# cggos/ptam_cg

Measured on AMD Instinct MI355X. Metric: BA LM iterations/s (50 KF x 5k pts) [+ tracked frames/s @640x480 in 'tracking'], higher is better.
Workload: dtype f64; 1 GPU; bundle_50kf_x_5000pts_dense; keyframes=50, points_total=5000, measurements_total=250000, measurements_rank0=250000, estimator=Tukey, parallelism=1 GPU, halfsample=R

## Files before the change

### ptam_cg_amd/csrc/ba_schur.inc

```
__device__ __forceinline__ void vinv_body(const BaDev& d, double lambda, int bx) {
    const int p = bx * 256 + threadIdx.x;
    if (p >= d.P) return;
    double v[6];
    const int r0 = d.rowptr[p], r1 = d.rowptr[p + 1];
    const int c0 = r0 >> 6, c1 = (r1 - 1) >> 6;
    if (d.cut != nullptr && r1 > r0 && c0 != c1) {
        const double* q = d.cut + (size_t)(2 * c0 + 1) * 9;
        double e[3] = {q[6], q[7], q[8]};
#pragma unroll
        for (int i = 0; i < 6; i++) v[i] = q[i];
        for (int c = c0 + 1; c <= c1; c++) {
            q = d.cut + (size_t)(2 * c) * 9;
#pragma unroll
            for (int i = 0; i < 6; i++) v[i] += q[i];
#pragma unroll
            for (int i = 0; i < 3; i++) e[i] += q[6 + i];
        }
#pragma unroll
        for (int i = 0; i < 3; i++) d.epsB[(size_t)p * 3 + i] = e[i];
    } else {
#pragma unroll
        for (int i = 0; i < 6; i++) v[i] = d.V[(size_t)p * 6 + i];
    }
    double A[9] = {v[0], v[1], v[3], v[1], v[2], v[4], v[3], v[4], v[5]};
    double* out = d.Vinv + (size_t)p * 9;
    if (A[0] * A[4] * A[8] == 0) {
#pragma unroll
        for (int i = 0; i < 9; i++) out[i] = 0;
        return;
    }
    A[0] *= (1.0 + lambda);
    A[4] *= (1.0 + lambda);
    A[8] *= (1.0 + lambda);
    for (int col = 0; col < 3; col++) {
        double inv_diag = 1;
        for (int row = col; row < 3; row++) {
            double val = A[row * 3 + col];
            for (int c2 = 0; c2 < col; c2++) val -= A[c2 * 3 + col] * A[row * 3 + c2];
            if (row == col) {
                A[row * 3 + col] = val;
                inv_diag = 1 / val;
            } else {
                A[col * 3 + row] = val;
                A[row * 3 + col] = val * inv_diag;
            }
        }
    }
    for (int c = 0; c < 3; c++) {
        double y[3], x[3];
        for (int i = 0; i < 3; i++) {
            double val = (i == c) ? 1.0 : 0.0;
            for (int j = 0; j < i; j++) val -= A[i * 3 + j] * y[j];
            y[i] = val;
        }
        for (int i = 0; i < 3; i++) y[i] /= A[i * 3 + i];
        for (int i = 2; i >= 0; i--) {
            double val = y[i];
            for (int j = i + 1; j < 3; j++) val -= A[j * 3 + i] * x[j];
            x[i] = val;
        }
        for (int r = 0; r < 3; r++) out[r * 3 + c] = x[r];
    }
}

__global__ void __launch_bounds__(256) vinv_kernel(BaDev d, double lambda) {
    TL_MARK(d, 6)
    if (ba_guard_blocks(d)) return;
    vinv_body(d, lambda, blockIdx.x);
}
__global__ void __launch_bounds__(256) reduce_vinv_kernel(BaDev d, int grid_acc, int nx, double lambda, double lambda_stay) {
    TL_MARK(d, 5)
    const int4 gf = ba_guard_load(d);
    if (ba_guard_blocks(d, gf)) return;
    if (ba_guard_stay(d, gf)) lambda = lambda_stay;
    const int b = blockIdx.x, nr = nx * RSPLIT;
    if (b < nr)
        reduce_partials_body(d, grid_acc, b % nx, b / nx);
    else
        vinv_body(d, lambda, b - nr);
}

#define SCHUR_TILE_ELEMS (SCHUR_TC * SCHUR_TC * 36 + SCHUR_TC * 6)
#ifndef SCHUR_RING
#define SCHUR_RING 2
#endif
#ifndef SCHUR_NW
#define SCHUR_NW 4
#endif
#define SCHUR_WG_PER_CU (8 / SCHUR_NW)
#define SCHUR_RED_BYTES ((SCHUR_NW / 2) * 40 * 64 * 8)
#define SCHUR_N_VARIANTS 6
#define SCHUR_MAP_WPT 8

struct SchurGrp {
    double wa[3][3];
    double wb[3][3];
    double vi[9];
    double eb[3];
    unsigned pm;
};
typedef double v4f64 __attribute__((ext_vector_type(4)));
typedef double schur_d2 __attribute__((ext_vector_type(2), aligned(8)));

template <int MODE>
__host__ __device__ __forceinline__ int schur_row(int t, int rid) {
    if (MODE == 1) return rid;
    if (t < 2) return 6 * (rid / 3) + 2 * (rid % 3) + t;
    const int q = 16 + (rid >> 1);
    return 6 * (q / 3) + 2 * (q % 3) + (rid & 1);
}
struct SchurLane {
    int hi4, sh4, hi2, sh2;
    unsigned o4, o2;
};
template <int MODE>
__device__ __forceinline__ SchurLane schur_lane(int l15) {
    SchurLane L;
    const int r0 = schur_row<MODE>(0, l15), r2 = MODE == 3 ? schur_row<3>(2, l15) : 0;
    const int s0 = r0 / 6, s2 = r2 / 6;
    L.hi4 = s0 >> 2, L.sh4 = 8 * (s0 & 3), L.o4 = 8u * (unsigned)(r0 - 6 * s0);
    L.hi2 = s2 >> 2, L.sh2 = 8 * (s2 & 3), L.o2 = 8u * (unsigned)(r2 - 6 * s2);
    return L;
}

__device__ __forceinline__ unsigned schur_slot_off(unsigned o0, unsigned o1, int first, int hi, int sh, int M, bool& present) {
    const unsigned o = ((hi ? o1 : o0) >> sh) & 0xffu;
    present = o != 0xffu;
    return (present ? (unsigned)first + o : (unsigned)M) * 48u;
}

template <int MODE>
__device__ __forceinline__ void schur_fetch_role(const char* __restrict__ W0, const char* __restrict__ W1, const char* __restrict__ W2,
// ... 494 lines not shown
```

### ptam_cg_amd/csrc/ba_update.inc

```
__global__ void __launch_bounds__(64) pose_update_kernel(BaDev d, int cur) {
    const int c = blockIdx.x * 64 + threadIdx.x;
    if (c < d.C) {
        const double* T = d.pose[cur] + 12 * c;
        double* Tn = d.pose[cur ^ 1] + 12 * c;
        const int f = d.cam_free[c];
        if (f < 0) {
#pragma unroll
            for (int i = 0; i < 12; i++) Tn[i] = T[i];
        } else {
            double mu[6], Tl[12], o[12];
#pragma unroll
            for (int i = 0; i < 6; i++) mu[i] = d.da[6 * f + i];
#pragma unroll
            for (int i = 0; i < 12; i++) Tl[i] = T[i];
            se3_exp_mul(mu, Tl, o);
#pragma unroll
            for (int i = 0; i < 12; i++) Tn[i] = o[i];
        }
    }
    if (blockIdx.x == 0) {
        double s = 0;
        for (int i = threadIdx.x; i < d.n; i += 64) s += d.da[i] * d.da[i];
        s = wave_sum_f64(s);
        if (threadIdx.x == 0) d.sumsq2[0] = s, d.sumsq2[1] = 0.0;
// ... 34 lines not shown
                t2 += w[(2 * h) * 3 + 2] * a0 + w[(2 * h + 1) * 3 + 2] * a1;
            }
        }
    }
    Ts[tid][0] = t0, Ts[tid][1] = t1, Ts[tid][2] = t2;
    __syncthreads();
    if (tid < 64) {
        double s0 = 0, s1 = 0, s2 = 0;
        for (int q = tid; q < BA_CHUNK; q += 64) s0 += Ts[q][0], s1 += Ts[q][1], s2 += Ts[q][2];
        s0 = wave_sum_f64(s0), s1 = wave_sum_f64(s1), s2 = wave_sum_f64(s2);
        if (tid == 0) {
            const double* eb = d.epsB + (size_t)pp * 3;
            const double* vi = d.Vinv + (size_t)pp * 9;
            const double* X = d.pt[cur] + (size_t)pp * 3;
            const double v0 = eb[0] - s0, v1 = eb[1] - s1, v2 = eb[2] - s2;
            const double d0 = vi[0] * v0 + vi[1] * v1 + vi[2] * v2, d1 = vi[3] * v0 + vi[4] * v1 + vi[5] * v2, d2 = vi[6] * v0 + vi[7] * v1 + vi[8] * v2;
            double* Xn = d.pt[cur ^ 1] + (size_t)pp * 3;
            Xn[0] = X[0] + d0, Xn[1] = X[1] + d1, Xn[2] = X[2] + d2;
            wred[0][0] = Xn[0], wred[0][1] = Xn[1], wred[1][0] = Xn[2], wred[1][1] = d0 * d0 + d1 * d1 + d2 * d2;
        }
    }
    __syncthreads();
    const double Xn[3] = {wred[0][0], wred[0][1], wred[1][0]};
    const double sq = wred[1][1];
    const double s2 = sig2;
    double err = 0;
    for (int m = ch.m_begin + tid; m < ch.m_end; m += BA_CHUNK) {
        if (d.m_state[m] == MS_DEAD) continue;
        BaProj pr;
        if (!ba_project(cam, d.pose[cur ^ 1] + 12 * d.m_cam[m], Xn, pr)) {
            err += 1.0;
            d.m_zbad_t[m] = 1;
        } else {
            const double2 fo = d.m_found[m];
            const double sn = d.m_s[m];
            const double ex = sn * (fo.x - pr.u), ey = sn * (fo.y - pr.v), e2n = ex * ex + ey * ey;
            err += ba_objective(est, e2n, s2, 1.0 / s2);
            d.m_e2t[m] = e2n;
            d.m_zbad_t[m] = 0;
        }
    }
    __syncthreads();
    err = wave_sum_f64(err);
    if ((tid & 63) == 0) wred[tid >> 6][0] = err;
    __syncthreads();
    if (tid == 0) {
        double e = 0;
        for (int i = 0; i < BA_CHUNK / 64; i++) e += wred[i][0];
        d.err_part[2 * blockIdx.x] = e;
        d.err_part[2 * blockIdx.x + 1] = sq;
    }
}

template <bool LOADW>
__global__ void __launch_bounds__(BA_CHUNK) point_update_kernel(DevCam cam, BaDev d, int cur, int est) {
    TL_MARK(d, 11)
    __shared__ double Ts[BA_CHUNK][3];
    __shared__ double Np[BA_CHUNK][3];
    __shared__ double wred[BA_CHUNK / 64][2];
    const int tid = threadIdx.x;
    const BaChunk ch = d.chunks[blockIdx.x];
    if (ch.m_end - ch.m_begin > BA_CHUNK) {
        point_update_long<LOADW>(cam, d, cur, est, ch, Ts, wred);
        return;
    }
    const int m = ch.m_begin + tid;
    const bool active = m < ch.m_end;
    const int mc = min(m, d.M - 1);
    const int st = active ? (int)d.m_state[mc] : (int)MS_DEAD;
    const int c = d.m_cam[mc], p = d.m_pt[mc];
    const int f = d.m_fidx[mc];
    const double s2 = d.sc->sigma_sq;
    const double2 fo = d.m_found[mc];
    const double sn = d.m_s[mc];
    const int npts = ch.pt_end - ch.pt_begin;
    const int pi0 = tid >> 3, sub = tid & 7;
    const bool on0 = pi0 < npts;
    const int pp0 = ch.pt_begin + (on0 ? pi0 : 0);
    const int rq0 = d.rowptr[pp0], rq1 = d.rowptr[pp0 + 1];
    double vi[9], x[3], eb[3];
    {
        const double* Vi = d.Vinv + (size_t)pp0 * 9;
        const double* X = d.pt[cur] + (size_t)pp0 * 3;
        const double* E = d.epsB + (size_t)pp0 * 3;
#pragma unroll
        for (int i = 0; i < 9; i++) vi[i] = Vi[i];
#pragma unroll
        for (int i = 0; i < 3; i++) x[i] = X[i], eb[i] = E[i];
    }
    double w[18];
    if (LOADW) {
        const size_t wp = w_plane(d);
#pragma unroll
        for (int c3 = 0; c3 < 3; c3++)
#pragma unroll
            for (int h = 0; h < 3; h++) {
                const double2 t = *(const double2*)(d.W + c3 * wp + (size_t)mc * 6 + 2 * h);
                w[(2 * h) * 3 + c3] = t.x;
                w[(2 * h + 1) * 3 + c3] = t.y;
            }
    }
    double da[6], T[12], Tc[12], xm[3];
    {
        const double2* dq = (const double2*)(d.da + 6 * (size_t)max(f, 0));
        const double2* Tq = (const double2*)(d.pose[cur ^ 1] + 12 * (size_t)c);
        if (!LOADW) {
            const double2* Cq = (const double2*)(d.pose[cur] + 12 * (size_t)c);
            const double* Xm = d.pt[cur] + (size_t)p * 3;
#pragma unroll
            for (int i = 0; i < 6; i++) {
                const double2 t = Cq[i];
                Tc[2 * i] = t.x, Tc[2 * i + 1] = t.y;
            }
#pragma unroll
            for (int i = 0; i < 3; i++) xm[i] = Xm[i];
        }
#pragma unroll
        for (int i = 0; i < 3; i++) {
            const double2 t = dq[i];
            da[2 * i] = t.x, da[2 * i + 1] = t.y;
        }
        if (LOADW) {
#pragma unroll
            for (int i = 0; i < 6; i++) {
                const double2 t = Tq[i];
                T[2 * i] = t.x, T[2 * i + 1] = t.y;
            }
        }
    }
    double t0 = 0, t1 = 0, t2 = 0;
    if (st == MS_ALIVE && f >= 0) {
        if (!LOADW) ba_rebuild_w(cam, est, Tc, xm, fo, sn, s2, w);
#pragma unroll
        for (int r = 0; r < 6; r++) {
            const double a = da[r];
            t0 += w[r * 3] * a;
            t1 += w[r * 3 + 1] * a;
            t2 += w[r * 3 + 2] * a;
        }
    }
    if (!LOADW) {
        const double2* Tq = (const double2*)(d.pose[cur ^ 1] + 12 * (size_t)c);
#pragma unroll
        for (int i = 0; i < 6; i++) {
            const double2 t = Tq[i];
            T[2 * i] = t.x, T[2 * i + 1] = t.y;
        }
    }
    Ts[tid][0] = t0;
    Ts[tid][1] = t1;
    Ts[tid][2] = t2;
    __syncthreads();
    double sq = 0;
    for (int base = 0; base < npts; base += BA_CHUNK / 8) {
        const int pi = base + pi0;
        const bool on = pi < npts;
        const int pp = ch.pt_begin + (on ? pi : 0);
        int r0 = rq0 - ch.m_begin, r1 = on0 ? rq1 - ch.m_begin : r0;
        if (base != 0) {
            r0 = d.rowptr[pp] - ch.m_begin, r1 = on ? d.rowptr[pp + 1] - ch.m_begin : r0;
            const double* Vi = d.Vinv + (size_t)pp * 9;
            const double* X = d.pt[cur] + (size_t)pp * 3;
            const double* E = d.epsB + (size_t)pp * 3;
#pragma unroll
            for (int i = 0; i < 9; i++) vi[i] = Vi[i];
#pragma unroll
            for (int i = 0; i < 3; i++) x[i] = X[i], eb[i] = E[i];
        }
        const double e0 = eb[0], e1 = eb[1], e2 = eb[2];
        double s0 = 0, s1 = 0, s2 = 0;
        for (int rr = r0 + sub; rr < r1; rr += 8) {
            s0 += Ts[rr][0];
            s1 += Ts[rr][1];
            s2 += Ts[rr][2];
        }
        s0 += dpp_row_shr_f64<1>(s0), s1 += dpp_row_shr_f64<1>(s1), s2 += dpp_row_shr_f64<1>(s2);
        s0 += dpp_row_shr_f64<2>(s0), s1 += dpp_row_shr_f64<2>(s1), s2 += dpp_row_shr_f64<2>(s2);
        s0 += dpp_row_shr_f64<4>(s0), s1 += dpp_row_shr_f64<4>(s1), s2 += dpp_row_shr_f64<4>(s2);
        if (on && sub == 7) {
            const double v0 = e0 - s0, v1 = e1 - s1, v2 = e2 - s2;
            const double d0 = vi[0] * v0 + vi[1] * v1 + vi[2] * v2;
            const double d1 = vi[3] * v0 + vi[4] * v1 + vi[5] * v2;
            const double d2 = vi[6] * v0 + vi[7] * v1 + vi[8] * v2;
            sq += d0 * d0 + d1 * d1 + d2 * d2;
            const double n0 = x[0] + d0, n1 = x[1] + d1, n2 = x[2] + d2;
            double* Xn = d.pt[cur ^ 1] + (size_t)pp * 3;
            Xn[0] = n0;
            Xn[1] = n1;
            Xn[2] = n2;
            Np[pi][0] = n0;
            Np[pi][1] = n1;
            Np[pi][2] = n2;
        }
    }
    __syncthreads();
// ... 179 lines not shown
```

### ptam_cg_amd/csrc/bundle.h

```cpp
#pragma once
#include <cstddef>

#include "common.h"
#include "map_stage.h"

enum { MS_ALIVE = 0, MS_BAD = 1, MS_DEAD = 2 };

#define BA_CHUNK 256
#define SCHUR_TC 8
#define SOLVE_NB 32
#define HIST_BINS 4096

struct BaChunk {
    int pt_begin, pt_end, m_begin, m_end;
};

struct SchurEntry {
    int pt;
    int ma;
    int mb;
    int pad;
    unsigned offa[2];
    unsigned offb[2];
};
struct SchurWG {
    int pair;
    int e_begin, e_end;
    int slot;
};

struct BaScalars {
    double sigma_sq;
    double cur_err;
    double new_err;
    double sumsq_cam;
    double sumsq_pt;
    double median;
    long long n_valid;
    int n_bad;
    int n_outliers;
    int sel_bin;
    int sel_k;
    int n_cand;
    int sel_bin2;
    int sel_k2;
    int select_overflow;
    int n_outliers_pub;
    int pad_;
    int end_step;
    int spec_go;
    int spec_stay;
    int spec_seq;
    int abort_any;
    int solve_fault;
};
static_assert(offsetof(BaScalars, end_step) % 16 == 0 && sizeof(BaScalars) % 8 == 0, "BaScalars: the decision words are read as one 16-byte load");

struct BaDev {
    int C, F, P, M;
    int guard;
    int guard_seq;
    int n, npad;
    int band;
    int n_chunks, grid_acc;
    int u_rows;
    int n_wchunks;
    int n_tiles, n_pairs, n_schur_wg, n_schur_entries;
    double* pose[2];
    int* cam_free;
    double* pt[2];
    double* V;
    double* epsB;
    double* Vinv;
    double* cut;
    int* rowptr;
    int* m_cam;
    int* m_pt;
    double2* m_found;
    double* m_s;
    int* m_orig;
    int* m_fidx;
    uint8_t* m_state;
    double* m_e2;
    double* m_e2t;
    uint8_t* m_zbad_t;
    double* W;
    double* Usplit;
    double* Upart;
    double* Adet;
    int* cam_ptr;
    int* cam_meas;
    double* err_part;
    int* bad_part;
    BaChunk* chunks;
    BaChunk* wchunks;
    unsigned* hist;
    double* cand;
    SchurEntry* s_entries;
    SchurWG* s_segs;
    int* s_wg_seg;
    int* s_pair_wg_begin;
    int* s_wg_head;
    double* s_part;
    unsigned* s_map;
    double* SE;
    double* L;
    double* Dg;
    double* y;
    double* da;
    double *SE2, *L2, *Dg2, *y2;
    unsigned* sflags2;
    unsigned* sflags;
    unsigned solve_seq;
    int chain_off;
    int chain_xcd;
    int spin_limit;
    double* bw_scratch;
    double* sumsq2;
    int* outliers;
    BaScalars* sc;
    long long* dbg;
};

__host__ __device__ __forceinline__ size_t w_plane(const BaDev& d) { return (size_t)(d.M + 1) * 6; }

__host__ __device__ __forceinline__ size_t se_blocks_before_row(int bi, int band) {
// ... 57 lines not shown
```

### ptam_cg_amd/csrc/bundle.hip

```cpp
#include <algorithm>
#include <array>
#include <chrono>
#include <climits>
#include <limits>
#include <atomic>
#include <numeric>
#include <utility>

#include "bundle.h"
#include "wait_mapped.h"
#include "../../include/ptam_hip_bench.h"

#include "ba_math.inc"
#include "ba_pass1.inc"
#include "ba_select.inc"
#include "ba_jacobian.inc"
#include "ba_schur.inc"
#include "ba_update.inc"
#include "ba_prepare.inc"

template <class T>
struct PinVec {
    ptam_ctx* ctx = nullptr;
    T* p = nullptr;
// ... 423 lines not shown
    const int n64 = (p.M + 63) / 64;
    const size_t lds_max = 160 * 1024;
    K7Launch k;
    bool loop = use_wave && n64 > 256 * 24;
    if (const char* e = ptam_ab_env("PTAM_K7_LOOP")) loop = use_wave && atoi(e) != 0;
    if (int rc = ba_k7_rules(ba, p, loop, k)) return rc;
    if (use_wave && k.loop && !k.big) {
        if (const char* e = ptam_ab_env("PTAM_K7_THREADS")) {
            const int t = atoi(e);
            if ((t == 256 || t == 512 || t == 1024) && !(k.det && t != 256) && ba_k7_smem(k, p, t) <= lds_max) {
                k.threads = t;
                if (int rc = ba_k7_per_cu(ba, p, k, t, &k.per_cu)) return rc;
                k.per_cu = std::max(1, std::min(k.per_cu, 8));
            }
        }
        if (const char* e = ptam_ab_env("PTAM_K7_WG_PER_CU")) k.per_cu = std::max(1, std::min(k.per_cu, atoi(e)));
    }
    if (use_wave && !k.loop) {
        if (const char* e = ptam_ab_env("PTAM_K7_THREADS1")) {
            const int t = atoi(e);
            if ((t == 512 || t == 1024) && !(k.det && t != 1024) && ba_k7_smem(k, p, t) <= lds_max) {
                k.threads = t;
                if (int rc = ba_k7_per_cu(ba, p, k, t, &k.per_cu)) return rc;
            }
        }
    }
    k.smem = ba_k7_smem(k, p, k.threads);
    if (use_wave) {
        const int wpb = k.threads / 64;
        if (k.loop) {
            const int n_cu = ba->ctx->n_cu > 0 ? ba->ctx->n_cu : 256;
            k.grid = std::max(1, std::min(n_cu * k.per_cu, n64 / wpb));
            const int waves = k.grid * wpb;
            k.per_wave = n64 / waves;
            k.extra_waves = n64 - k.per_wave * waves;
        } else
            k.grid = std::max(1, (n64 + wpb - 1) / wpb);
    }
    k.u_rows = k.det ? p.n_dtiles : (k.big || !use_wave) ? 1 : k.grid;
    *out = k;
    return PTAM_OK;
}

static void ba_layout_main(Carver& cv, const ptam_ba* ba, BaDev& d, Prep& p) {
    PrepDev& q = p.q;
    const bool det = ba->k7.det;
    const size_t Mz = std::max(p.M, 1), Pz = std::max(p.P_all, 1), Cz = std::max(p.C, 1), Fz = std::max(p.F, 1), Maz = std::max(p.Mall, 1);
    const size_t n_dtiles = (size_t)p.n_dtiles;
    (void)cv.take(Cz * 96);
    d.pose[1] = cv.piece<double>(Cz * 12);
    d.pt[0] = cv.piece<double>(Pz * 3), d.pt[1] = cv.piece<double>(Pz * 3);
    d.V = cv.piece<double>(Pz * 6);
    d.epsB = cv.piece<double>(Pz * 3);
    d.Vinv = cv.piece<double>(Pz * 9);
    d.rowptr = cv.piece<int>(Pz + 1);
    d.cut = cv.piece<double>(ba->use_wave ? (size_t)((p.M + 63) / 64) * 2 * 9 : 1);
    if (!ba->use_wave) d.cut = nullptr;
    d.m_cam = cv.piece<int>(Mz), d.m_pt = cv.piece<int>(Mz);
    d.m_found = cv.piece<double2>(Mz);
    d.m_s = cv.piece<double>(Mz);
    d.m_orig = cv.piece<int>(Mz), d.m_fidx = cv.piece<int>(Mz);
    d.m_state = cv.piece<uint8_t>(Mz);
    d.m_e2 = cv.piece<double>(Mz), d.m_e2t = cv.piece<double>(Mz);
    d.m_zbad_t = cv.piece<uint8_t>(Mz);
    d.W = cv.piece<double>((Mz + 1) * 18);
    d.Usplit = cv.piece<double>(Fz * 27 * 16);
    d.Upart = cv.piece<double>((size_t)std::max(d.grid_acc, det ? p.n_dtiles : 1) * Fz * 27);
    d.Adet = cv.piece<double>(det ? Mz * 14 : 1);
    if (!det) d.Adet = nullptr;
    d.cam_ptr = cv.piece<int>(det ? n_dtiles * (Fz + 1) : 2), d.cam_meas = cv.piece<int>(det ? Mz : 2);
    p.tile_free = cv.piece<int>(det ? n_dtiles + 1 : 2);
    d.err_part = cv.piece<double>(std::max<size_t>(p.chunks_cap, (size_t)d.grid_acc) * 2 + 2);
    d.bad_part = cv.piece<int>((size_t)d.grid_acc + 4);
    d.chunks = cv.piece<BaChunk>(p.chunks_cap), d.wchunks = cv.piece<BaChunk>(1);
    d.hist = cv.piece<unsigned>(2 * HIST_BINS);
    d.cand = cv.piece<double>(Mz);
    const size_t npad = std::max(d.npad, SOLVE_NB), nblk = npad / SOLVE_NB;
    const size_t se_full = se_size((int)nblk, (int)nblk - 1), n_flags = ba_solve_flag_bytes((int)nblk) / sizeof(unsigned);
    d.SE = cv.piece<double>(se_full + npad + 8);
    d.L = cv.piece<double>(se_full);
    d.Dg = cv.piece<double>(npad), d.y = cv.piece<double>(npad), d.da = cv.piece<double>(npad);
    d.sumsq2 = cv.piece<double>(2);
    d.bw_scratch = cv.piece<double>(npad * 12);
    d.sflags = cv.piece<unsigned>(n_flags), d.sflags2 = cv.piece<unsigned>(n_flags);
    d.SE2 = cv.piece<double>(se_full + npad + 8);
    d.L2 = cv.piece<double>(se_full);
    d.Dg2 = cv.piece<double>(npad), d.y2 = cv.piece<double>(npad);
    d.outliers = cv.piece<int>(Mz);
    d.sc = cv.piece<BaScalars>(1), d.dbg = cv.piece<long long>(8192);
    p.xchg = cv.piece<double>(512);
    const size_t hist_n = (size_t)8 * std::max(p.n_pairs, 1) * 16;
    q.cnt = cv.piece<int>(Pz);
    q.tcode = cv.piece<unsigned long long>(Pz * (size_t)p.nw);
    q.hist = cv.piece<int>(hist_n);
    p.clear_bytes = cv.off;
    p.small = cv.piece<char>(p.small_bytes);
    Carver sm{p.small};
    const PrepSmall s = ba_layout_small(sm, Cz, p.pair_order.size());
    q.ps = s.ps, d.pose[0] = s.pose, d.cam_free = s.cam_free, q.pair_order = s.pair_order;
    p.r_dead = cv.piece<uint8_t>(Maz);
    p.pts_raw = cv.piece<double>(Pz * 3);
    q.start = cv.piece<int>(Pz + 1), q.dense_of = cv.piece<int>(Pz);
    q.pt_orig = cv.piece<int>(Pz);
    q.arr = cv.piece<int>(Maz);
    q.tmp_i = cv.piece<int>(Mz), q.tmp_key = cv.piece<int>(Mz);
    q.ptile = cv.piece<int4>(Mz);
    q.kp = cv.piece<int>(Pz), q.costp = cv.piece<int>(Pz);
// ... 461 lines not shown
            hipLaunchKernelGGL(unpack2_kernel, dim3(1), dim3(1), 0, ctx->stream, d.sc, (const double*)ba->d_xchg, 0);
        }
    }
    return PTAM_OK;
}

static int ba_ensure_mailbox(ptam_ba* ba) {
    if (ba->mbox) return PTAM_OK;
    void* h = nullptr;
    size_t cap = 0;
    if (int rc = ctx_block_take(ba->ctx, CTX_MEM_MAPPED, sizeof(ptam_ba::Mailbox), &h, &cap)) return rc;
    std::memset(h, 0, sizeof(ptam_ba::Mailbox));
    void* dv = nullptr;
    HIP_TRY(hipHostGetDevicePointer(&dv, h, 0));
    ba->mbox = (ptam_ba::Mailbox*)h;
    ba->mbox_dev = (ptam_ba::Mailbox*)dv;
    return PTAM_OK;
}

static int ba_trial(ptam_ba* ba, double lambda, bool skip_vinv, int last_allowed, int abort_local, bool decide_in_prologue = false) {
    ptam_ctx* ctx = ba->ctx;
    BaDev& d = ba->d;
    prof_begin(ba, PTAM_K_VINV);
    if (d.P > 0 && !skip_vinv) hipLaunchKernelGGL(vinv_kernel, dim3((d.P + 255) / 256), dim3(256), 0, ctx->stream, d, lambda);
    prof_end(ba, PTAM_K_VINV);
    if (d.F > 0) {
        prof_begin(ba, PTAM_K_SCHUR);
        if (d.n_schur_wg > 0)
            hipLaunchKernelGGL(schur_tile_mfma_kernel, dim3(d.n_schur_wg), dim3(64 * SCHUR_NW), SCHUR_RED_BYTES, ctx->stream, d);
        hipLaunchKernelGGL(schur_reduce_kernel, dim3(d.n_pairs, SRED_SLICES), dim3(256), 0, ctx->stream, d, lambda,
                           (ba->world > 1 && ba->rank != 0) ? 0 : 1);
        prof_end(ba, PTAM_K_SCHUR);
        HIP_TRY(hipGetLastError());
        const size_t n_se = se_size(d.npad / SOLVE_NB, se_band(d)) + d.npad;
        const bool sharded = ba->comm && ba->world > 1;
        if (sharded) prof_begin(ba, PTAM_K_EXCHANGE);
        int rc = ba_allreduce(ba, d.SE, n_se + (ba->cur_pending ? 2 : 0));
        if (sharded) prof_end(ba, PTAM_K_EXCHANGE);
        if (rc) return rc;
        if (ba->cur_pending) {
            hipLaunchKernelGGL(unpack2_kernel, dim3(1), dim3(1), 0, ctx->stream, d.sc, (const double*)(d.SE + n_se), 0);
            ba->cur_pending = false;
        }
        prof_begin(ba, PTAM_K_SOLVE);
        rc = ba_solve(ctx, d, ba->cur);
        prof_end(ba, PTAM_K_SOLVE);
        if (rc) return rc;
    }
    prof_begin(ba, PTAM_K_UPDATE);
    if (d.F == 0)
        hipLaunchKernelGGL(pose_update_kernel, dim3(std::max(1, (d.C + 63) / 64)), dim3(64), 0, ctx->stream, d, ba->cur);
    if (d.n_chunks > 0) {
        static const bool loads_w = getenv("PTAM_UPDATE_LOADS_W") != nullptr;
        hipLaunchKernelGGL(loads_w ? point_update_kernel<true> : point_update_kernel<false>, dim3(d.n_chunks), dim3(BA_CHUNK), 0,
                           ctx->stream, ctx->cam, d, ba->cur, ba->opts.estimator);
    }
    {
        const bool fuse = !(ba->comm && ba->world > 1) && !ba->prof;
        ulonglong2* slots = nullptr;
        unsigned long long seq = 0;
        if (fuse) {
            const int rcm = ba_ensure_mailbox(ba);
            if (rcm) return rcm;
            slots = (ulonglong2*)ba->mbox_dev;
            seq = ++ba->mbox_seq;
            ba->published_by_finalize = true;
        }
        ba->decide_pending = decide_in_prologue;
        ba->decide_last_allowed = last_allowed;
        if (!decide_in_prologue)
            hipLaunchKernelGGL(finalize_new_kernel, dim3(1), dim3(256), 0, ctx->stream, d, ba->opts.update_sq_conv_limit, last_allowed,
                               slots, seq);
    }
    prof_end(ba, PTAM_K_UPDATE);
    HIP_TRY(hipGetLastError());
    if (ba->comm && ba->world > 1) {
        hipLaunchKernelGGL(pack2_kernel, dim3(1), dim3(1), 0, ctx->stream, (const BaScalars*)d.sc, ba->d_xchg, 1, abort_local);
        int rc = ba_allreduce(ba, ba->d_xchg, 4);
        if (rc) return rc;
        hipLaunchKernelGGL(unpack2_kernel, dim3(1), dim3(1), 0, ctx->stream, d.sc, (const double*)ba->d_xchg, 1);
    }
    return PTAM_OK;
}

static int ba_p1_blocks() {
    static const int n = [] {
        const char* e = ptam_ab_env("PTAM_P1_BLOCKS");
        return e ? std::max(1, atoi(e)) : 512;
    }();
    return n;
}
static int ba_enqueue_speculative(ptam_ba* ba, double lambda_next, double lambda_stay) {
    ptam_ctx* ctx = ba->ctx;
    BaDev d = ba->d;
    const double min_s2 = ba->opts.min_sigma * ba->opts.min_sigma;
    d.guard = 1;
    d.guard_seq = (int)ba->mbox_seq;
    const dim3 g_p1(std::max(1, std::min((d.M + 256 * P1_U - 1) / (256 * P1_U), ba_p1_blocks())));
    if (ba->decide_pending) {
        hipLaunchKernelGGL(purge_pass1_decide_kernel, g_p1, dim3(256), 0, ctx->stream, d, ba->opts.update_sq_conv_limit, ba->decide_last_allowed,
                           (ulonglong2*)ba->mbox_dev, ba->mbox_seq);
        ba->decide_pending = false;
    } else
        hipLaunchKernelGGL(purge_pass1_kernel, g_p1, dim3(256), 0, ctx->stream, d);
    hipLaunchKernelGGL(select_compact_kernel, dim3(std::max(1, std::min((d.M + 1023) / 1024, ba_sel_blocks()))), dim3(256), 0, ctx->stream, d,
                       (const double*)d.m_e2, (long long)d.M, (const uint8_t*)d.m_state, 0);
    hipLaunchKernelGGL(select_final_kernel, dim3(1), dim3(1024), 0, ctx->stream, d, ba->opts.estimator, min_s2);
    launch_k7(ba, 1);
    {
        const int nx = std::max(1, (d.F * 27 + 63) / 64);
        hipLaunchKernelGGL(reduce_vinv_kernel, dim3(nx * RSPLIT + (d.P + 255) / 256), dim3(256), 0, ctx->stream, d, d.grid_acc, nx,
                           lambda_next, lambda_stay);
    }
    HIP_TRY(hipGetLastError());
    return PTAM_OK;
}

static int ba_publish_scalars(ptam_ba* ba) {
    ptam_ctx* ctx = ba->ctx;
    int rc = ba_ensure_mailbox(ba);
    if (rc) return rc;
    if (ba->published_by_finalize) {
        ba->published_by_finalize = false;
        return PTAM_OK;
    }
    const unsigned long long seq = ++ba->mbox_seq;
    hipLaunchKernelGGL(publish_scalars_kernel, dim3(1), dim3(64), 0, ctx->stream, (const BaScalars*)ba->d.sc,
                       (ulonglong2*)ba->mbox_dev, seq);
    HIP_TRY(hipGetLastError());
    return PTAM_OK;
}

static int ba_wait_scalars(ptam_ba* ba, BaScalars* out) {
    ptam_ctx* ctx = ba->ctx;
    const unsigned long long seq = ba->mbox_seq;
    constexpr unsigned NW = sizeof(BaScalars) / 8;
    auto arrived = [&]() {
        for (unsigned i = 0; i < NW; i++)
            if (ba->mbox->slot[i].seq != seq) return false;
        return true;
    };
    if (ba->prof) {
        HIP_TRY(ptam_stream_wait(ctx->stream));
    } else {
        const int rc = ptam_wait_mapped(ctx->stream, "a trial's scalars", arrived, [&](bool drained) {
            if (!ba_debug().wait) return;
            std::fprintf(stderr, "[ptam] waiting for seq %llu: stream %s, slots", seq, drained ? "drained" : "busy");
            for (unsigned i = 0; i < NW; i++) std::fprintf(stderr, " %llu", (unsigned long long)ba->mbox->slot[i].seq);
            std::fprintf(stderr, "\n");
        });
        if (rc) return rc;
    }
    unsigned long long words[NW];
    for (;;) {
        std::atomic_thread_fence(std::memory_order_acquire);
        for (unsigned i = 0; i < NW; i++) words[i] = ba->mbox->slot[i].v;
        std::atomic_thread_fence(std::memory_order_acquire);
        if (arrived()) break;
    }
    std::memcpy(out, words, sizeof(BaScalars));
    prof_collect(ba);
    return PTAM_OK;
}

static int ba_read_scalars(ptam_ba* ba, BaScalars* out) {
// ... 299 lines not shown
    if (ba->d_sel && world != ba->world) {
        HIP_TRY(hipSetDevice(ba->ctx->device));
        HIP_TRY(ptam_stream_wait(ba->ctx->stream));
        HIP_TRY(hipFree(ba->d_sel));
        ba->d_sel = nullptr;
    }
    ba->rank = rank;
    ba->world = world;
    ba->comm = fn;
    ba->comm_user = user;
    return PTAM_OK;
}

#define BA_DBG(...) do { if (dbg.wait) { std::fprintf(stderr, "[ptam] " __VA_ARGS__); std::fprintf(stderr, "\n"); } } while (0)
int ptam_ba_compute(ptam_ba* ba, const volatile unsigned char* abort_flag, int* accepted_out) {
    ARG_TRY(ba);
    ptam_ctx* ctx = ba->ctx;
    const BaDebug& dbg = ba_debug();
    HIP_TRY(hipSetDevice(ctx->device));
    BA_DBG("compute: prepare");
    const bool sharded = ba->comm && ba->world > 1;
    int rc = ptam_ba_prepare(ba);
    if (rc && !sharded) return rc;
    const int rc_prepare = rc;
    BA_DBG("compute: prepared M=%d P=%d F=%d chunks=%d wchunks=%d grid_acc=%d schur_wg=%d", ba->d.M, ba->d.P, ba->d.F, ba->d.n_chunks,
           ba->d.n_wchunks, ba->d.grid_acc, ba->d.n_schur_wg);
    BaDev& d = ba->d;
    ChainTurn chain_turn(d, ctx->device);
    double lambda = 0.0001, lambda_factor = 2.0;
    ba->converged = ba->published_by_finalize = ba->cur_pending = ba->slow_select = false;
    ba->trial_is_current = ba->e2_is_current = false;
    bool hit_max = false;
    int counter = 0;
    ba->accepted = 0;
    ba->trials.clear();
    std::vector<int> step_outlier_end;
    int n_steps = 0;
    bool prev_end_pending = false;
    bool abort_all = false;
    auto abort_local = [&]() { return abort_flag && *abort_flag; };
    auto aborted = [&]() { return sharded ? abort_all : abort_local(); };
    BaScalars sc;
    std::memset(&sc, 0, sizeof sc);
    double dbg_enq_ms = 0, dbg_wait_ms = 0;
    std::vector<double> trial_read_us;
    const auto dbg_t0 = std::chrono::steady_clock::now();
    BaHostTimes ht;
    ba_dbg_begin(ba, ht);
    if (sharded && (rc = ba_sharded_handshake(ba, rc_prepare, abort_local(), &abort_all, chain_turn))) return rc;
    const bool empty = d.M == 0;
    const bool spec = !sharded && !ba->prof && d.n_chunks > 0 && !ptam_ab_env("PTAM_NO_SPECULATION");
    bool spec_ready = false;
    const bool fused_decision = !ptam_ab_env("PTAM_SEPARATE_FINALIZE");
    while (!empty && !ba->converged && !hit_max && !aborted()) {
        bool skip_vinv = false;
        if (spec_ready) {
            spec_ready = false;
            skip_vinv = true;
        } else {
            if ((rc = ba_pass1_sigma(ba))) return rc;
            if ((rc = ba_pass2(ba))) return rc;
        }
        bool have_cur = false;
        double cur_err = 0, new_err = 0;
        bool ran_any = false, redo_step = false, nan_stop = false;
        for (;;) {
            if (have_cur && !(new_err > cur_err)) break;
            if (ba->converged || hit_max || aborted()) break;
            BA_DBG("trial %d lambda %g", counter, lambda);
            const auto q0 = std::chrono::steady_clock::now();
            rc = ba_trial(ba, lambda, skip_vinv, counter + 1 >= ba->opts.max_iterations ? 1 : 0, abort_local() ? 1 : 0, spec && fused_decision);
            dbg_enq_ms += ba_stall_ms(q0, counter, "took", "to enqueue");
            skip_vinv = false;
            if (rc) return rc;
            if ((rc = ba_publish_scalars(ba))) return rc;
            if (spec) {
                if ((rc = ba_enqueue_speculative(ba, lambda * 0.3, lambda))) return rc;
            }
            BA_DBG("trial %d enqueued, waiting", counter);
            const auto w0 = std::chrono::steady_clock::now();
            rc = ba_wait_scalars(ba, &sc);
            dbg_wait_ms += ba_stall_ms(w0, counter, "waited", "for its scalars");
            if (rc) return rc;
            BA_DBG("trial %d read: cur %g new %g sigma2 %g median %g n_valid %lld n_bad %d sumsq %g %g", counter, sc.cur_err, sc.new_err,
                   sc.sigma_sq, sc.median, sc.n_valid, sc.n_bad, sc.sumsq_cam, sc.sumsq_pt);
            ba_dbg_first_read(ht);
            if (!have_cur) {
                if (prev_end_pending) step_outlier_end.push_back(spec && fused_decision ? sc.n_outliers_pub : sc.n_outliers);
                prev_end_pending = false;
                if (sc.select_overflow && !ba->slow_select) {
                    ba->slow_select = true;
                    if (dbg.select) std::fprintf(stderr, "[ptam] rank %d: select overflow, repeating the step on the gather path\n", ba->rank);
                    redo_step = true;
                    break;
                }
                have_cur = true;
                cur_err = sc.cur_err;
                new_err = cur_err + 9999;
                if (!(new_err > cur_err)) {
                    nan_stop = true;
                    break;
                }
            }
            if (sc.solve_fault) {
                if ((rc = ba_solve_fallback(ba, counter))) return rc;
                continue;
            }
            ran_any = true;
            if (dbg.trial_times) trial_read_us.push_back(std::chrono::duration<double, std::micro>(std::chrono::steady_clock::now() - dbg_t0).count());
            if (sharded) abort_all = abort_all || sc.abort_any != 0;
            new_err = sc.new_err;
            const double sumsq = sc.sumsq_cam + sc.sumsq_pt;
            if (sumsq < ba->opts.update_sq_conv_limit) ba->converged = true;
            ptam_ba_trial t;
            t.lambda = lambda;
            t.sigma_sq = sc.sigma_sq;
            t.err_old = cur_err;
            t.err_new = new_err;
            t.sum_sq_update = sumsq;
            t.n_bad = sc.n_bad;
            t.accepted = 0;
            if (ba->opts.verbose)
                std::printf("L%.1e\tOld %.6f  New %.6f  Diff %.6f\n", lambda, cur_err, new_err, cur_err - new_err);
            if (new_err > cur_err) {
                lambda = lambda * lambda_factor;
                lambda_factor = lambda_factor * 2;
            }
            counter++;
            if (counter >= ba->opts.max_iterations) hit_max = true;
            ba->trials.push_back(t);
        }
        if (redo_step) continue;
        if (nan_stop) hit_max = true;
        ba->trial_is_current = false;
        ba->e2_is_current = ran_any && !(new_err < cur_err);
        if (ran_any && new_err < cur_err) {
            lambda_factor = 2.0;
            lambda *= 0.3;
            ba->cur ^= 1;
            ba->accepted++;
            ba->trials.back().accepted = 1;
            ba->trial_is_current = true;
        }
        if (prev_end_pending) {
            if ((rc = ba_read_scalars(ba, &sc))) return rc;
            step_outlier_end.push_back(sc.n_outliers);
        }
        const bool stayed = spec && ran_any && !(new_err < cur_err) && !(new_err > cur_err) && !ba->converged && !hit_max;
        spec_ready = (spec && ran_any && new_err < cur_err && !ba->converged && !hit_max) || stayed;
        if (!spec_ready && d.M > 0)
            hipLaunchKernelGGL(purge_kernel, dim3((d.M + 255) / 256), dim3(256), 0, ctx->stream, d);
        prev_end_pending = true;
        HIP_TRY(hipGetLastError());
        n_steps++;
    }
    BA_DBG("loop done, steps %d", n_steps);
    ba_report_trial_times(ba, trial_read_us);
    if (dbg.stall)
        std::fprintf(stderr, "[ptam] compute loop: %zu trials in %.3f ms; host enqueueing trials %.3f ms, waiting for scalars %.3f ms\n",
                     ba->trials.size(), std::chrono::duration<double, std::milli>(std::chrono::steady_clock::now() - dbg_t0).count(),
                     dbg_enq_ms, dbg_wait_ms);
    if (n_steps > 0) {
        if ((rc = ba_read_scalars(ba, &sc))) return rc;
        step_outlier_end.push_back(sc.n_outliers);
    }
    if ((rc = ba_dbg_loop_end(ba, ht))) return rc;
    const int n_out = step_outlier_end.empty() ? 0 : step_outlier_end.back();
    std::vector<int> out_idx(std::max(n_out, 1));
    if ((rc = ba_readback(ba, n_out, out_idx))) return rc;
    ba->raw_out.insert(ba->raw_out.end(), out_idx.begin(), out_idx.begin() + n_out);
    for (int end : step_outlier_end) ba->raw_out_ends.push_back(ba->raw_out_base + end);
    ba->raw_out_base += n_out;
    if (n_out > 0) ba->prepared = false;
    if ((rc = ba_dbg_dump(ba, ht))) return rc;
    if (dbg.stall)
        std::fprintf(stderr, "[ptam] compute total %.3f ms\n",
                     std::chrono::duration<double, std::milli>(std::chrono::steady_clock::now() - dbg_t0).count());
    if (accepted_out) *accepted_out = ba->accepted;
    return PTAM_OK;
}

int ptam_ba_converged(const ptam_ba* ba) { return ba && ba->converged ? 1 : 0; }

int ptam_ba_get_point(const ptam_ba* ba, int n, double pos[3]) {
    ARG_TRY(ba && pos && n >= 0 && n < (int)(ba->pts.size() / 3));
    std::memcpy(pos, &ba->pts[3 * (size_t)n], 24);
    return PTAM_OK;
}
int ptam_ba_get_camera(const ptam_ba* ba, int n, double pose[12]) {
    ARG_TRY(ba && pose && n >= 0 && n < (int)ba->cam_fixed.size());
    std::memcpy(pose, &ba->cam_pose[12 * (size_t)n], 96);
    return PTAM_OK;
}
int ptam_ba_get_all(const ptam_ba* ba, double* poses12, double* points3) {
    ARG_TRY(ba);
    if (poses12) std::memcpy(poses12, ba->cam_pose.data(), ba->cam_pose.size() * 8);
    if (points3) std::memcpy(points3, ba->pts.data(), ba->pts.size() * 8);
    return PTAM_OK;
}
int ptam_ba_get_outliers(const ptam_ba* ba, int32_t* pairs, int cap) {
    if (!ba) return PTAM_E_ARG;
    ba_finish_outliers(const_cast<ptam_ba*>(ba));
// ... 203 lines not shown
        if (rc) return rc;
        ARG_TRY(bas[i]->d.M > 0);
        rc = ba_pass1_sigma(bas[i]);
        if (rc) return rc;
    }
    for (int r = 0; r < 2; r++)
        for (int i = 0; i < n; i++) launch_k7(bas[i]);
    HIP_TRY(ptam_stream_wait(ctx->stream));
    hipEvent_t e0, e1;
    HIP_TRY(hipEventCreate(&e0));
    HIP_TRY(hipEventCreate(&e1));
    HIP_TRY(hipEventRecord(e0, ctx->stream));
    for (int r = 0; r < reps; r++)
        for (int i = 0; i < n; i++) launch_k7(bas[i]);
    HIP_TRY(hipEventRecord(e1, ctx->stream));
    HIP_TRY(hipEventSynchronize(e1));
    float ms_total = 0;
    HIP_TRY(hipEventElapsedTime(&ms_total, e0, e1));
    hipEventDestroy(e0);
    hipEventDestroy(e1);
    *avg_ms = (double)ms_total / ((double)reps * n);
    return PTAM_OK;
}

}

int ba_preload_kernels() {
    ptam_preload((const void*)project_e2_kernel);
    ptam_preload((const void*)pass1_from_trial_kernel);
    ptam_preload((const void*)pass1_keep_kernel);
    ptam_preload((const void*)purge_pass1_kernel);
    ptam_preload((const void*)purge_pass1_decide_kernel);
    ptam_preload((const void*)hist_keys_kernel);
    ptam_preload((const void*)select_compact_kernel);
    ptam_preload((const void*)select_final_kernel);
    ptam_preload((const void*)hist_to_f64_kernel);
    ptam_preload((const void*)f64_to_hist_kernel);
    ptam_preload((const void*)select_stage_kernel);
    ptam_preload((const void*)select_finish_kernel);
    ptam_preload((const void*)compact_valid_kernel);
    ptam_preload(k7_wave_fn(256, true, -1, true));
    for (int est : {(int)PTAM_EST_TUKEY, (int)PTAM_EST_CAUCHY})
        for (int lp = 0; lp < 2; lp++) ptam_preload(k7_wave_fn(lp ? 256 : 1024, lp != 0, est, false, true));
    ptam_preload(k7_wave_fn(256, true, -1, true, true));
    ptam_preload((const void*)reduce_det_kernel);
    ptam_preload((const void*)reduce_partials_kernel);
    ptam_preload((const void*)vinv_kernel);
    ptam_preload((const void*)reduce_vinv_kernel);
    ptam_preload((const void*)schur_tile_mfma_kernel);
    ptam_preload((const void*)schur_reduce_kernel);
    ptam_preload((const void*)pose_update_kernel);
    ptam_preload((const void*)point_update_kernel<false>);
    ptam_preload((const void*)point_update_kernel<true>);
    ptam_preload((const void*)finalize_new_kernel);
    ptam_preload((const void*)purge_kernel);
    ptam_preload((const void*)readback_kernel);
    ptam_preload((const void*)stamp_kernel);
    ptam_preload((const void*)publish_scalars_kernel);
    ptam_preload((const void*)set_scalars_kernel);
    ptam_preload((const void*)set_new_kernel);
    ptam_preload((const void*)pack2_kernel);
    ptam_preload((const void*)unpack2_kernel);
    ptam_preload((const void*)place_keys_kernel);
    for (int est = 0; est < 2; est++) {
        ptam_preload(k7_wave_fn(512, false, est ? PTAM_EST_CAUCHY : PTAM_EST_TUKEY));
        ptam_preload(k7_wave_fn(1024, false, est ? PTAM_EST_CAUCHY : PTAM_EST_TUKEY));
        ptam_preload(k7_wave_fn(256, true, est ? PTAM_EST_CAUCHY : PTAM_EST_TUKEY));
        ptam_preload(k7_wave_fn(512, true, est ? PTAM_EST_CAUCHY : PTAM_EST_TUKEY));
        ptam_preload(k7_wave_fn(1024, true, est ? PTAM_EST_CAUCHY : PTAM_EST_TUKEY));
    }
    HIP_TRY(hipFuncSetAttribute((const void*)reduce_det_kernel, hipFuncAttributeMaxDynamicSharedMemorySize, (int)((size_t)14 * (DET_TILE + 1) * sizeof(double))));
    HIP_TRY(hipFuncSetAttribute((const void*)schur_tile_mfma_kernel, hipFuncAttributeMaxDynamicSharedMemorySize, SCHUR_RED_BYTES));
    return PTAM_OK;
}
```

Before: 6944 LM iterations/s.

## Precompute retry-lambda Vinv speculatively and stage poses in LDS for point update

The speculative reduce_vinv launch now also inverts the point blocks for the lambda a rejected trial would retry with, writing them into a second Vinv buffer. The host swaps that buffer in when the retry matches, so the vinv pass is skipped on a rejection. Separately, point_update_kernel gains a variant that copies all camera poses, updated poses, camera deltas and the chunk's points into LDS before the per-measurement gathers. This costs extra blocks and memory per speculative step plus an added barrier and dynamic LDS in the update kernel.

```diff
diff --git a/ptam_cg_amd/csrc/ba_schur.inc b/ptam_cg_amd/csrc/ba_schur.inc
--- a/ptam_cg_amd/csrc/ba_schur.inc
+++ b/ptam_cg_amd/csrc/ba_schur.inc
@@ -1,34 +1,5 @@
-__device__ __forceinline__ void vinv_body(const BaDev& d, double lambda, int bx) {
-    const int p = bx * 256 + threadIdx.x;
-    if (p >= d.P) return;
-    double v[6];
-    const int r0 = d.rowptr[p], r1 = d.rowptr[p + 1];
-    const int c0 = r0 >> 6, c1 = (r1 - 1) >> 6;
-    if (d.cut != nullptr && r1 > r0 && c0 != c1) {
-        const double* q = d.cut + (size_t)(2 * c0 + 1) * 9;
-        double e[3] = {q[6], q[7], q[8]};
-#pragma unroll
-        for (int i = 0; i < 6; i++) v[i] = q[i];
-        for (int c = c0 + 1; c <= c1; c++) {
-            q = d.cut + (size_t)(2 * c) * 9;
-#pragma unroll
-            for (int i = 0; i < 6; i++) v[i] += q[i];
-#pragma unroll
-            for (int i = 0; i < 3; i++) e[i] += q[6 + i];
-        }
-#pragma unroll
-        for (int i = 0; i < 3; i++) d.epsB[(size_t)p * 3 + i] = e[i];
-    } else {
-#pragma unroll
-        for (int i = 0; i < 6; i++) v[i] = d.V[(size_t)p * 6 + i];
-    }
+__device__ __forceinline__ void vinv_invert(const double (&v)[6], double lambda, double (&out)[9]) {
     double A[9] = {v[0], v[1], v[3], v[1], v[2], v[4], v[3], v[4], v[5]};
-    double* out = d.Vinv + (size_t)p * 9;
-    if (A[0] * A[4] * A[8] == 0) {
-#pragma unroll
-        for (int i = 0; i < 9; i++) out[i] = 0;
-        return;
-    }
     A[0] *= (1.0 + lambda);
     A[4] *= (1.0 + lambda);
     A[8] *= (1.0 + lambda);
@@ -62,22 +33,61 @@
         for (int r = 0; r < 3; r++) out[r * 3 + c] = x[r];
     }
 }
+__device__ __forceinline__ void vinv_body(const BaDev& d, double lambda, int bx, double* __restrict__ Vout, bool own_epsb = true) {
+    const int p = bx * 256 + threadIdx.x;
+    if (p >= d.P) return;
+    double v[6];
+    const int r0 = d.rowptr[p], r1 = d.rowptr[p + 1];
+    const int c0 = r0 >> 6, c1 = (r1 - 1) >> 6;
+    if (d.cut != nullptr && r1 > r0 && c0 != c1) {
+        const double* q = d.cut + (size_t)(2 * c0 + 1) * 9;
+        double e[3] = {q[6], q[7], q[8]};
+#pragma unroll
+        for (int i = 0; i < 6; i++) v[i] = q[i];
+        for (int c = c0 + 1; c <= c1; c++) {
+            q = d.cut + (size_t)(2 * c) * 9;
+#pragma unroll
+            for (int i = 0; i < 6; i++) v[i] += q[i];
+#pragma unroll
+            for (int i = 0; i < 3; i++) e[i] += q[6 + i];
+        }
+        if (own_epsb) {
+#pragma unroll
+            for (int i = 0; i < 3; i++) d.epsB[(size_t)p * 3 + i] = e[i];
+        }
+    } else {
+#pragma unroll
+        for (int i = 0; i < 6; i++) v[i] = d.V[(size_t)p * 6 + i];
+    }
+    double* out = Vout + (size_t)p * 9;
+    double x[9];
+    if (v[0] * v[2] * v[5] == 0) {
+#pragma unroll
+        for (int i = 0; i < 9; i++) x[i] = 0;
+    } else
+        vinv_invert(v, lambda, x);
+#pragma unroll
+    for (int i = 0; i < 9; i++) out[i] = x[i];
+}
 
 __global__ void __launch_bounds__(256) vinv_kernel(BaDev d, double lambda) {
     TL_MARK(d, 6)
     if (ba_guard_blocks(d)) return;
-    vinv_body(d, lambda, blockIdx.x);
-}
-__global__ void __launch_bounds__(256) reduce_vinv_kernel(BaDev d, int grid_acc, int nx, double lambda, double lambda_stay) {
+    vinv_body(d, lambda, blockIdx.x, d.Vinv);
+}
+__global__ void __launch_bounds__(256) reduce_vinv_kernel(BaDev d, int grid_acc, int nx, double lambda, double lambda_stay, double retry,
+                                                          double retry_stay) {
     TL_MARK(d, 5)
     const int4 gf = ba_guard_load(d);
     if (ba_guard_blocks(d, gf)) return;
-    if (ba_guard_stay(d, gf)) lambda = lambda_stay;
-    const int b = blockIdx.x, nr = nx * RSPLIT;
+    if (ba_guard_stay(d, gf)) lambda = lambda_stay, retry = retry_stay;
+    const int b = blockIdx.x, nr = nx * RSPLIT, nv = (d.P + 255) / 256;
     if (b < nr)
         reduce_partials_body(d, grid_acc, b % nx, b / nx);
+    else if (b < nr + nv)
+        vinv_body(d, lambda, b - nr, d.Vinv);
     else
-        vinv_body(d, lambda, b - nr);
+        vinv_body(d, retry, b - nr - nv, d.Vinv2, false);
 }
 
 #define SCHUR_TILE_ELEMS (SCHUR_TC * SCHUR_TC * 36 + SCHUR_TC * 6)
diff --git a/ptam_cg_amd/csrc/ba_update.inc b/ptam_cg_amd/csrc/ba_update.inc
--- a/ptam_cg_amd/csrc/ba_update.inc
+++ b/ptam_cg_amd/csrc/ba_update.inc
@@ -110,14 +110,29 @@
     }
 }
 
-template <bool LOADW>
+#define PU_LDS_MAX_CAMS ((2 * BA_CHUNK) / 6)
+template <bool LOADW, bool LDSP = false>
 __global__ void __launch_bounds__(BA_CHUNK) point_update_kernel(DevCam cam, BaDev d, int cur, int est) {
     TL_MARK(d, 11)
+    static_assert(!(LOADW && LDSP), "the staged form rebuilds W");
     __shared__ double Ts[BA_CHUNK][3];
     __shared__ double Np[BA_CHUNK][3];
     __shared__ double wred[BA_CHUNK / 64][2];
+    extern __shared__ __attribute__((aligned(16))) double pu_tab[];
     const int tid = threadIdx.x;
     const BaChunk ch = d.chunks[blockIdx.x];
+    const int n6 = d.C * 6, nf3 = d.F * 3;
+    double2 tv[5];
+    if (LDSP) {
+        const double2* Pc = (const double2*)d.pose[cur];
+        const double2* Pt = (const double2*)d.pose[cur ^ 1];
+        const double2* Dq = (const double2*)d.da;
+        tv[0] = Pc[min(tid, n6 - 1)];
+        tv[1] = Pc[min(tid + BA_CHUNK, n6 - 1)];
+        tv[2] = Pt[min(tid, n6 - 1)];
+        tv[3] = Pt[min(tid + BA_CHUNK, n6 - 1)];
+        tv[4] = Dq[max(min(tid, nf3 - 1), 0)];
+    }
     if (ch.m_end - ch.m_begin > BA_CHUNK) {
         point_update_long<LOADW>(cam, d, cur, est, ch, Ts, wred);
         return;
@@ -159,7 +174,35 @@
             }
     }
     double da[6], T[12], Tc[12], xm[3];
-    {
+    const double2* tab = (const double2*)pu_tab;
+    if (LDSP) {
+        const double* Xq = d.pt[cur] + (size_t)(ch.pt_begin + max(min(tid, npts - 1), 0)) * 3;
+        const double q0 = Xq[0], q1 = Xq[1], q2 = Xq[2];
+        double2* tw = (double2*)pu_tab;
+        const int spare = 2 * n6 + nf3;
+        tw[tid < n6 ? tid : spare] = tv[0];
+        tw[tid + BA_CHUNK < n6 ? tid + BA_CHUNK : spare] = tv[1];
+        tw[tid < n6 ? n6 + tid : spare] = tv[2];
+        tw[tid + BA_CHUNK < n6 ? n6 + tid + BA_CHUNK : spare] = tv[3];
+        tw[tid < nf3 ? 2 * n6 + tid : spare] = tv[4];
+        Np[tid][0] = q0, Np[tid][1] = q1, Np[tid][2] = q2;
+        __syncthreads();
+        const double2* Cq = tab + 6 * c;
+        const double2* dq = tab + 2 * n6 + 3 * max(f, 0);
+        const double* Xm = Np[active ? p - ch.pt_begin : 0];
+#pragma unroll
+        for (int i = 0; i < 6; i++) {
+            const double2 t = Cq[i];
+            Tc[2 * i] = t.x, Tc[2 * i + 1] = t.y;
+        }
+#pragma unroll
+        for (int i = 0; i < 3; i++) xm[i] = Xm[i];
+#pragma unroll
+        for (int i = 0; i < 3; i++) {
+            const double2 t = dq[i];
+            da[2 * i] = t.x, da[2 * i + 1] = t.y;
+        }
+    } else {
         const double2* dq = (const double2*)(d.da + 6 * (size_t)max(f, 0));
         const double2* Tq = (const double2*)(d.pose[cur ^ 1] + 12 * (size_t)c);
         if (!LOADW) {
@@ -198,7 +241,7 @@
         }
     }
     if (!LOADW) {
-        const double2* Tq = (const double2*)(d.pose[cur ^ 1] + 12 * (size_t)c);
+        const double2* Tq = LDSP ? tab + n6 + 6 * c : (const double2*)(d.pose[cur ^ 1] + 12 * (size_t)c);
 #pragma unroll
         for (int i = 0; i < 6; i++) {
             const double2 t = Tq[i];
diff --git a/ptam_cg_amd/csrc/bundle.h b/ptam_cg_amd/csrc/bundle.h
--- a/ptam_cg_amd/csrc/bundle.h
+++ b/ptam_cg_amd/csrc/bundle.h
@@ -72,6 +72,7 @@
     double* V;
     double* epsB;
     double* Vinv;
+    double* Vinv2;
     double* cut;
     int* rowptr;
     int* m_cam;
diff --git a/ptam_cg_amd/csrc/bundle.hip b/ptam_cg_amd/csrc/bundle.hip
--- a/ptam_cg_amd/csrc/bundle.hip
+++ b/ptam_cg_amd/csrc/bundle.hip
@@ -499,7 +499,7 @@
     d.pt[0] = cv.piece<double>(Pz * 3), d.pt[1] = cv.piece<double>(Pz * 3);
     d.V = cv.piece<double>(Pz * 6);
     d.epsB = cv.piece<double>(Pz * 3);
-    d.Vinv = cv.piece<double>(Pz * 9);
+    d.Vinv = cv.piece<double>(Pz * 9), d.Vinv2 = cv.piece<double>(Pz * 9);
     d.rowptr = cv.piece<int>(Pz + 1);
     d.cut = cv.piece<double>(ba->use_wave ? (size_t)((p.M + 63) / 64) * 2 * 9 : 1);
     if (!ba->use_wave) d.cut = nullptr;
@@ -1067,8 +1067,13 @@
         hipLaunchKernelGGL(pose_update_kernel, dim3(std::max(1, (d.C + 63) / 64)), dim3(64), 0, ctx->stream, d, ba->cur);
     if (d.n_chunks > 0) {
         static const bool loads_w = getenv("PTAM_UPDATE_LOADS_W") != nullptr;
-        hipLaunchKernelGGL(loads_w ? point_update_kernel<true> : point_update_kernel<false>, dim3(d.n_chunks), dim3(BA_CHUNK), 0,
-                           ctx->stream, ctx->cam, d, ba->cur, ba->opts.estimator);
+        static const bool global_poses = getenv("PTAM_UPDATE_GLOBAL_POSES") != nullptr;
+        if (!loads_w && !global_poses && d.C <= PU_LDS_MAX_CAMS)
+            hipLaunchKernelGGL((point_update_kernel<false, true>), dim3(d.n_chunks), dim3(BA_CHUNK),
+                               ((size_t)12 * d.C + 3 * d.F + 1) * 16, ctx->stream, ctx->cam, d, ba->cur, ba->opts.estimator);
+        else
+            hipLaunchKernelGGL(loads_w ? point_update_kernel<true> : point_update_kernel<false>, dim3(d.n_chunks), dim3(BA_CHUNK), 0,
+                               ctx->stream, ctx->cam, d, ba->cur, ba->opts.estimator);
     }
     {
         const bool fuse = !(ba->comm && ba->world > 1) && !ba->prof;
@@ -1105,7 +1110,7 @@
     }();
     return n;
 }
-static int ba_enqueue_speculative(ptam_ba* ba, double lambda_next, double lambda_stay) {
+static int ba_enqueue_speculative(ptam_ba* ba, double lambda_next, double lambda_stay, bool retry_prep, double retry_next, double retry_stay) {
     ptam_ctx* ctx = ba->ctx;
     BaDev d = ba->d;
     const double min_s2 = ba->opts.min_sigma * ba->opts.min_sigma;
@@ -1124,8 +1129,8 @@
     launch_k7(ba, 1);
     {
         const int nx = std::max(1, (d.F * 27 + 63) / 64);
-        hipLaunchKernelGGL(reduce_vinv_kernel, dim3(nx * RSPLIT + (d.P + 255) / 256), dim3(256), 0, ctx->stream, d, d.grid_acc, nx,
-                           lambda_next, lambda_stay);
+        hipLaunchKernelGGL(reduce_vinv_kernel, dim3(nx * RSPLIT + (retry_prep ? 2 : 1) * ((d.P + 255) / 256)), dim3(256), 0, ctx->stream, d,
+                           d.grid_acc, nx, lambda_next, lambda_stay, retry_next, retry_stay);
     }
     HIP_TRY(hipGetLastError());
     return PTAM_OK;
@@ -1531,8 +1536,13 @@
     const bool spec = !sharded && !ba->prof && d.n_chunks > 0 && !ptam_ab_env("PTAM_NO_SPECULATION");
     bool spec_ready = false;
     const bool fused_decision = !ptam_ab_env("PTAM_SEPARATE_FINALIZE");
+    static const bool retry_launch = getenv("PTAM_RETRY_VINV_LAUNCH") != nullptr;
+    const bool retry_prep = spec && !retry_launch && d.P > 0;
+    double spec_retry_go = 0, spec_retry_stay = 0, prepared_lambda = 0;
     while (!empty && !ba->converged && !hit_max && !aborted()) {
         bool skip_vinv = false;
+        bool prepared_retry = spec_ready && retry_prep;
+        int trials_in_step = 0;
         if (spec_ready) {
             spec_ready = false;
             skip_vinv = true;
@@ -1548,13 +1558,19 @@
             if (ba->converged || hit_max || aborted()) break;
             BA_DBG("trial %d lambda %g", counter, lambda);
             const auto q0 = std::chrono::steady_clock::now();
+            if (prepared_retry && trials_in_step == 1 && lambda == prepared_lambda) {
+                std::swap(d.Vinv, d.Vinv2);
+                skip_vinv = true;
+            }
+            if (trials_in_step >= 1) prepared_retry = false;
             rc = ba_trial(ba, lambda, skip_vinv, counter + 1 >= ba->opts.max_iterations ? 1 : 0, abort_local() ? 1 : 0, spec && fused_decision);
             dbg_enq_ms += ba_stall_ms(q0, counter, "took", "to enqueue");
             skip_vinv = false;
             if (rc) return rc;
             if ((rc = ba_publish_scalars(ba))) return rc;
             if (spec) {
-                if ((rc = ba_enqueue_speculative(ba, lambda * 0.3, lambda))) return rc;
+                spec_retry_go = (lambda * 0.3) * 2.0, spec_retry_stay = lambda * lambda_factor;
+                if ((rc = ba_enqueue_speculative(ba, lambda * 0.3, lambda, retry_prep, spec_retry_go, spec_retry_stay))) return rc;
             }
             BA_DBG("trial %d enqueued, waiting", counter);
             const auto w0 = std::chrono::steady_clock::now();
@@ -1606,6 +1622,7 @@
                 lambda_factor = lambda_factor * 2;
             }
             counter++;
+            trials_in_step++;
             if (counter >= ba->opts.max_iterations) hit_max = true;
             ba->trials.push_back(t);
         }
@@ -1627,6 +1644,7 @@
         }
         const bool stayed = spec && ran_any && !(new_err < cur_err) && !(new_err > cur_err) && !ba->converged && !hit_max;
         spec_ready = (spec && ran_any && new_err < cur_err && !ba->converged && !hit_max) || stayed;
+        prepared_lambda = stayed ? spec_retry_stay : spec_retry_go;
         if (!spec_ready && d.M > 0)
             hipLaunchKernelGGL(purge_kernel, dim3((d.M + 255) / 256), dim3(256), 0, ctx->stream, d);
         prev_end_pending = true;
@@ -1936,6 +1954,7 @@
     ptam_preload((const void*)pose_update_kernel);
     ptam_preload((const void*)point_update_kernel<false>);
     ptam_preload((const void*)point_update_kernel<true>);
+    ptam_preload((const void*)point_update_kernel<false, true>);
     ptam_preload((const void*)finalize_new_kernel);
     ptam_preload((const void*)purge_kernel);
     ptam_preload((const void*)readback_kernel);
```

After: 7008 LM iterations/s, median of 6. About the same (+0.9%).
